# rounak-meyur/revs-admm

Measured on NVIDIA B200. Metric: home_hours_scheduled_per_sec, higher is better.
Workload: dtype f64

## Files before the change

revs-admm_b200/csrc/dual_update.cu:

```cuda
#include <cuda_bf16.h>

#include "kernels.cuh"

namespace revs {



__device__ __forceinline__ unsigned long long ld_acquire_sys(const unsigned long long* p) {
    unsigned long long v;
    asm volatile("ld.acquire.sys.global.u64 %0, [%1];" : "=l"(v) : "l"(p) : "memory");
    return v;
}
__device__ __forceinline__ void st_release_sys(unsigned long long* p, unsigned long long v) {
    asm volatile("st.release.sys.global.u64 [%0], %1;" ::"l"(p), "l"(v) : "memory");
}

template <int SLOTS, bool DSUM>
__global__ void __launch_bounds__(256, 4) dual_update_kernel(DualParams P) {
    extern __shared__ double tile[];
    __shared__ double s_part[2][8];
    const int lane = threadIdx.x & 31, warp = threadIdx.x >> 5;
    const int h0 = blockIdx.x * 32;
    const int ldt = P.T + 1;
    const int it = P.iter ? *P.iter : 0;
    const double* __restrict__ p_sch_new = (it & 1) ? P.p_sch_old : P.p_sch_new;
    const double* __restrict__ p_sch_old = (it & 1) ? P.p_sch_new : P.p_sch_old;
    double* __restrict__ diff_k = P.diff_k + (size_t)it * P.Hp;

    {
        const int h = h0 + lane;
        const bool in = h < P.Hp;
        const double* src = P.g_t + (in ? h : 0);
        int t = warp;
        for (; t + 24 < P.T; t += 32) {
            double v[4];
#pragma unroll
            for (int q = 0; q < 4; ++q) v[q] = in ? src[(size_t)(t + 8 * q) * P.Hp] : 0.0;
#pragma unroll
            for (int q = 0; q < 4; ++q) tile[lane * ldt + t + 8 * q] = v[q];
        }
        for (; t < P.T; t += 8) tile[lane * ldt + t] = in ? src[(size_t)t * P.Hp] : 0.0;
    }
    __syncthreads();

    const double hk = 0.5 * P.kappa;
    double blk_p = 0.0, blk_d = 0.0;
    const double* dsum = DSUM ? P.dsum : nullptr;
    if constexpr (SLOTS > 0) {
        for (int hl = warp; hl < 32; hl += 16) {
            double sn[2][SLOTS], gm[2][SLOTS], so[2][DSUM ? 1 : SLOTS];
            bool okh[2];
#pragma unroll
            for (int q = 0; q < 2; ++q) {
                const int h = h0 + hl + 8 * q;
                okh[q] = h < P.Hp;
                const size_t base = (size_t)(okh[q] ? h : 0) * P.T;
#pragma unroll
                for (int j = 0; j < SLOTS; ++j) {
// ... 59 lines not shown
            blk_p += a1;
            blk_d += a2;
        }
    }
    if (lane == 0) { s_part[0][warp] = blk_p; s_part[1][warp] = blk_d; }
    __syncthreads();

    __nv_bfloat16* gbf = reinterpret_cast<__nv_bfloat16*>(P.gbf_next);
    for (int t = warp; t < P.T; t += 8) {
        int h = h0 + lane;
        if (h < P.Hp) {
            const double zv = tile[lane * ldt + t];
            const size_t o = (size_t)t * P.Hp + h;
            P.z_t[o] = zv;
            if (P.g_next) {
                const double gv = fmax(zv, 0.0);
                P.g_next[o] = gv;
                if (gbf) gbf[o] = __float2bfloat16_rn((float)gv);
            }
        }
    }

    __shared__ int s_last;
    __shared__ double s_fin[2][8];
    if (threadIdx.x == 0) {
        double sp = 0.0, sd = 0.0;
        for (int w = 0; w < 8; ++w) { sp += s_part[0][w]; sd += s_part[1][w]; }
        P.partials[blockIdx.x] = sp;
        P.partials[gridDim.x + blockIdx.x] = sd;
        __threadfence();
        const unsigned done = atomicAdd(&P.res->ticket, 1u);
// ... 46 lines not shown
        if (P.peer.world > 1) {
            count = 0.0;
            for (int r = 0; r < P.peer.world; ++r) { tp += s_peer[0][r]; td += s_peer[1][r]; count += s_peer[2][r]; }
        } else {
            for (int w = 0; w < 8; ++w) { tp += s_fin[0][w]; td += s_fin[1][w]; }
        }
        const double r = sqrt(tp / count), sres = P.kappa * sqrt(td / count);
        const int conv = (P.tol > 0.0 && r < P.tol && sres < P.tol) ? 1 : 0;
        P.res->sum_primal = tp;
        P.res->sum_dual = td;
        P.res->count = count;
        P.res->primal = r;
        P.res->dual = sres;
        P.res->converged = conv;
        P.res->ticket = 0u;
        if (P.iter) {
            const int k = it + 1;
            *P.iter = k;
            if (P.use_cond) {
                const bool err = (P.err_a && *P.err_a) || (P.err_b && *P.err_b) || (P.peer.world > 1 && *P.peer.timeout);
                cudaGraphSetConditional((cudaGraphConditionalHandle)P.cond_loop, (k < P.iter_max && !conv && !err) ? 1u : 0u);
            }
        }
    }
}

cudaError_t launch_dual_update(const DualParams& P, cudaStream_t stream) {
    const size_t smem = (size_t)32 * (P.T + 1) * sizeof(double);
    const int slots = (P.T + 31) / 32;
    const dim3 grid((P.Hp + 31) / 32);
    auto go = [&](auto kernel) -> cudaError_t {
        if (smem > 48 * 1024) {
            cudaError_t e = cudaFuncSetAttribute(kernel, cudaFuncAttributeMaxDynamicSharedMemorySize, (int)smem);
            if (e != cudaSuccess) return e;
        }
        kernel<<<grid, 256, smem, stream>>>(P);
        return cudaGetLastError();
    };
    if (P.dsum) {
        switch (slots) {
            case 1: return go(dual_update_kernel<1, true>);
            case 2: return go(dual_update_kernel<2, true>);
            case 3: return go(dual_update_kernel<3, true>);
// ... 15 lines not shown
```

revs-admm_b200/csrc/home_solve.cu:

```cuda
#include <math_constants.h>

#include "kernels.cuh"

namespace revs {

constexpr int kMaxSlots = 8;
constexpr int kSelectRounds = 24;


template <int SLOTS>
__global__ void __launch_bounds__(256, SLOTS <= 3 ? 6 : 1) home_solve_kernel(HomeParams P) {
    const int lane = threadIdx.x & 31;
    const int h = blockIdx.x * (blockDim.x >> 5) + (threadIdx.x >> 5);
    if (h >= P.Hp) return;
    const size_t base = (size_t)h * P.T;
    const bool ev = P.has_ev[h] != 0;
    const double rate = P.rating[h];
    const int st = P.start[h], en = P.end[h];
    const int nmin = P.n_min[h], nmax = P.n_max[h];
    const bool odd = P.iter != nullptr && (*P.iter & 1);
    const double* __restrict__ p_sch_in = odd ? P.p_sch_new : P.p_sch;
    double* __restrict__ p_sch_out = odd ? const_cast<double*>(P.p_sch) : P.p_sch_new;

    double ld[SLOTS];
#pragma unroll
    for (int j = 0; j < SLOTS; ++j) {
        int t = lane + 32 * j;
        ld[j] = t < P.T ? P.load[base + t] : 0.0;
    }
    const bool first = P.iter ? (*P.iter == 0) : (P.first != 0);
    if (!ev) {
        double a2 = 0.0;
#pragma unroll
        for (int j = 0; j < SLOTS; ++j) {
            int t = lane + 32 * j;
            if (t < P.T) {
                p_sch_out[base + t] = ld[j];
                P.p_ev[base + t] = 0.0;
                const double ds = first ? ld[j] : 0.0;
                a2 = fma(ds, ds, a2);
            }
        }
        if (P.dsum) {
            a2 = warp_sum(a2);
            if (lane == 0) P.dsum[h] = a2;
// ... 99 lines not shown
#pragma unroll
                for (int j = 0; j < SLOTS; ++j) {
                    int t = lane + 32 * j;
                    rank[j] += (o < d[j]) || (o == d[j] && s < t);
                }
            }
        }
#pragma unroll
        for (int j = 0; j < SLOTS; ++j)
            on[j] = d[j] < CUDART_INF && (rank[j] < nmin || (rank[j] < nmax && d[j] < 0.0));
    }
    double a2 = 0.0;
#pragma unroll
    for (int j = 0; j < SLOTS; ++j) {
        int t = lane + 32 * j;
        if (t >= P.T) continue;
        double p = on[j] ? rate : 0.0;
        P.p_ev[base + t] = p;
        const double sn = __dadd_rn(ld[j], p);
        p_sch_out[base + t] = sn;
        const double ds = sn - prev[j];
        a2 = fma(ds, ds, a2);
    }
    if (P.dsum) {
        a2 = warp_sum(a2);
        if (lane == 0) P.dsum[h] = a2;
    }
}

cudaError_t launch_home_solve(const HomeParams& P, cudaStream_t stream) {
    const int warps = 8;
// ... 38 lines not shown
```

revs-admm_b200/csrc/kernels.cuh:

```cuda
#pragma once
#include <vector>

#include "common.cuh"

namespace revs {

struct HomeParams {
    const double* load;
    const double* p_est;
    const double* p_sch;
    const int* iter;
    const double* gamma;
    const double* cost;
    const uint8_t* has_ev;
    const double* rating;
    const int* start;
    const int* end;
    const int* n_min;
    const int* n_max;
    double* p_sch_new;
    double* p_ev;
    double* dsum;
    int first;
    int* infeasible;
    int Hp, T;
    double kappa;
    int individual;
    const double* ind_const;
};

cudaError_t launch_home_solve(const HomeParams& P, cudaStream_t stream);
cudaError_t launch_soc_profile(const double* p_ev, const uint8_t* has_ev, const double* capacity,
                               const double* initial, double* soc, int Hp, int T, cudaStream_t stream);

struct ResidualOut {
    double sum_primal;
    double sum_dual;
    double primal;
// ... 18 lines not shown
    const double* p_sch_old;
    const double* dsum;
    int* iter;
    int iter_max;
    int step;
    const int* err_a;
    const int* err_b;
    unsigned long long cond_loop;
    int use_cond;
    double* gamma;
    double* p_est;
    double* z_t;
    double* g_next;
    void* gbf_next;
    double* diff_k;
    ResidualOut* res;
    PeerReduce peer;
    double* partials;
    int Hp, T;
    double kappa, tol, count;
};

cudaError_t launch_dual_update(const DualParams& P, cudaStream_t stream);

struct QpParams {
    const FeederDev* feeders;
    const double* Rpool;
    const double* rn2;
    const double* rmax;
    int* cand;
// ... 51 lines not shown
cudaError_t launch_round_end(const RoundEndParams& P, cudaStream_t stream);

struct ClassGateParams {
    const int* order_count;
    unsigned long long cond[kQpClasses];
    int first_gated;
};
cudaError_t launch_class_gate(const ClassGateParams& P, cudaStream_t stream);
cudaError_t qp_warp_prepare();
cudaError_t screen_prepare();
cudaError_t screen_tc5_prepare();

cudaError_t launch_utility_qp(const QpParams& P, int grid, int cls, cudaStream_t stream);
int qp_warp_max_n();
cudaError_t launch_qp_init(const QpParams& P, int max_warp_n, cudaStream_t stream);
int qp_warp_ctas_per_sm();
int qp_warp_m_max_default();
cudaError_t launch_utility_qp_warp(const QpParams& P, int nj, int ctas_per_sm, cudaStream_t stream);
cudaError_t launch_utility_qp_fast(const QpParams& P, cudaStream_t stream);
cudaError_t launch_order_columns(const QpParams& P, int mode, int* order, int* order_count, cudaStream_t stream);

struct NewtonZone {
    int feeder;
    int nn, nlev, n;
    int wn;
    int col0;
    int64_t node_off;
    int64_t home_off;
    int64_t lvl_off;
    int64_t ws_off;
// ... 276 lines not shown
```

revs-admm_b200/csrc/revs_capi.cu:

```cuda
#include <chrono>
#include <cstdarg>
#include <cstdio>
#include <cstring>
#include <algorithm>
#include <cstdlib>
#include <cmath>
#include <mutex>
#include <string>
#include <vector>

#include "../../include/revs_admm.h"
#include "kernels.cuh"

using namespace revs;

namespace {

thread_local std::string g_err;

int fail(int code, const char* fmt, ...) {
    char buf[512];
    va_list ap;
    va_start(ap, fmt);
    vsnprintf(buf, sizeof buf, fmt, ap);
// ... 186 lines not shown
    double2* d_nt_ws2 = nullptr;
    int64_t nt_ws_stride = 0;
    int n_newton_cols = 0;
    size_t nt_sig = 0;
    double* d_gather = nullptr;
    int64_t gather_cap = 0;
    double* peer_gather[kGatherMaxPeers] = {};
    int gather_world = 1, gather_rank = 0;
    unsigned long long gather_seq = 0;
    GatherDev* d_gather_dev = nullptr;
    unsigned* d_gather_ticket = nullptr;
    int* d_gather_timeout = nullptr;
    bool use_warp_kernel = true;
    bool overlap_home = true;
    bool screen = true;
    int screen_impl = 0;
    void *d_maps_a = nullptr, *d_map_b = nullptr;
    int* d_bcol0 = nullptr;
    bool tc5_ready = false;
    int *d_pool_parent = nullptr, *d_pool_res = nullptr;
    double* d_pool_cumr = nullptr;
    int64_t* d_pool_off = nullptr;
    size_t pool_nodes = 0;
    NetTools net;
    size_t Rpool_elems = 0;
    bool rn2_valid = false;
    double *d_load = nullptr, *d_pest = nullptr, *d_psch[2] = {nullptr, nullptr}, *d_gamma = nullptr,
           *d_pev = nullptr, *d_soc = nullptr;
    uint8_t* d_has_ev = nullptr;
    double *d_rating = nullptr, *d_capacity = nullptr, *d_initial = nullptr, *d_indconst = nullptr;
// ... 548 lines not shown
        return fail(REVS_ERR_INFEASIBLE, "a home charging sub-problem is infeasible (SOC window vs plug-in window)");
    if (s->h_cnt->n_failed)
        return fail(REVS_ERR_NOCONV,
                    "utility QP: %d (feeder,hour) columns need more than %d simultaneously active "
                    "voltage rows", s->h_cnt->n_failed, kWMax);
    if (s->h_cnt->noconv)
        return fail(REVS_ERR_NOCONV, "utility QP: %d columns still running after %d working-set rounds (or a tree-Newton column "
                    "that did not reach the tolerance)", s->h_cnt->n_running, kQpRoundMax);
    return REVS_OK;
}

int utility_solve(revs_solver* s, bool in_loop = false) {
    int rc = prepare_sensitivity(s);
    if (rc) return rc;
    QpParams Q = qp_params(s);
    if ((rc = launch_init(s, Q, in_loop, true))) return rc;
    s->stats.kernel_launches++;
    if (newton_active(s)) {
        if ((rc = launch_newton_stage(s, true))) return rc;
        if (dense_cols(s) == 0) {
            CU(cudaMemcpyAsync(s->h_cnt, s->d_cnt, sizeof(Counters), cudaMemcpyDeviceToHost, s->sU));
            CU(cudaStreamSynchronize(s->sU));
            return check_device_flags(s);
        }
    }
    bool use[kQpClasses];
    for (int cl = 0; cl < kQpClasses; ++cl) use[cl] = cl <= 1 || qp_class_cap(cl - 1) < s->ws_bound;
    int top_cls = 0;
    int grid[kQpClasses];
    for (int cl = 0; cl < kQpClasses; ++cl) grid[cl] = s->ncols;
    for (int round = 0;; ++round) {
        if (round >= kQpRoundMax)
// ... 60 lines not shown
    P.rating = s->d_rating;
    P.start = s->d_start;
    P.end = s->d_end;
    P.n_min = individual ? s->d_zero_i : s->d_nmin;
    P.n_max = s->d_nmax;
    P.p_sch_new = s->d_psch[s->cur ^ 1];
    P.p_ev = s->d_pev;
    P.infeasible = &s->d_cnt->infeasible;
    P.Hp = (int)s->Hp;
    P.T = s->T;
    P.kappa = s->kappa;
    P.individual = individual;
    P.ind_const = s->d_indconst;
    P.dsum = nullptr;
    P.first = 0;
    return P;
}

void free_all(revs_solver* s) {
    cudaSetDevice(s->device);
    void* ptrs[] = {s->d_feeders, s->d_Rpool, s->d_rn2, s->d_rmax, s->d_cand, s->d_stage, s->d_hmap, s->d_Rbf, s->d_gbf, s->d_v32, s->d_sprob, s->d_stiles, s->d_maps_a, s->d_map_b, s->d_bcol0, s->d_pool_parent, s->d_pool_res, s->d_pool_cumr, s->d_pool_off, s->d_load, s->d_pest, s->d_psch[0], s->d_psch[1], s->d_gamma,
                    s->d_pev, s->d_soc, s->d_has_ev, s->d_rating, s->d_capacity, s->d_initial, s->d_indconst,
                    s->d_start, s->d_end, s->d_nmin, s->d_nmax, s->d_zero_i, s->d_cost, s->d_zt, s->d_lamt,
                    s->d_gt, s->d_vt, s->d_wcount, s->d_widx, s->d_status, s->d_innerok, s->d_cls, s->d_order, s->d_order4, s->d_order_count, s->d_cnt, s->d_diff,
                    s->d_cprob, s->d_ctiles, s->d_respart, s->d_dsum,
                    s->d_nt_zones, s->d_nt_lvl, s->d_nt_parent, s->d_nt_home, s->d_nt_hnode, s->d_nt_wsi, s->d_nt_child, s->d_nt_homes, s->d_nt_rho,
                    s->d_nt_ws, s->d_nt_ws4, s->d_nt_ws2};
    for (int r = 0; r < kMaxPeers; ++r)
        if (s->peer_box[r] && s->peer_box[r] != s->d_mailbox) cudaIpcCloseMemHandle(s->peer_box[r]);
    for (int r = 0; r < kGatherMaxPeers; ++r)
// ... 462 lines not shown
    D.cond_loop = 0;
    D.use_cond = 0;
    D.partials = s->d_respart;
    D.dsum = s->d_dsum;
    D.peer.world = s->comm_world;
    D.peer.rank = s->comm_rank;
    for (int r = 0; r < kMaxPeers; ++r) D.peer.box[r] = s->peer_box[r];
    D.peer.run_seq = s->d_run_seq;
    D.peer.timeout = s->d_comm_timeout;
    D.gamma = s->d_gamma;
    D.p_est = s->d_pest;
    D.z_t = s->d_zt;
    D.g_next = s->d_gt;
    D.gbf_next = s->screen ? s->d_gbf : nullptr;
    D.diff_k = s->d_diff;
    D.res = &s->d_cnt->res;
    D.Hp = (int)s->Hp;
    D.T = s->T;
    D.kappa = s->kappa;
    D.tol = s->tol;
    D.count = (double)s->H * s->T;
    return D;
}

int finish_sync(revs_solver* s, double sums[3]) {
    CU(cudaStreamSynchronize(s->sU));
    CU(cudaStreamSynchronize(s->sH));
    spans_collect(s);
    int rc = check_device_flags(s);
    if (rc == REVS_OK && s->comm_world > 1) {
// ... 17 lines not shown
        sums[2] = s->comm_world > 1 ? s->h_cnt->res.count : (double)s->H * s->T;
    }
    return REVS_OK;
}

int admm_step_impl(revs_solver* s, double sums[3], bool sync_now) {
    if (!s || !s->running) return fail(REVS_ERR_ARG, "revs_admm_begin has not been called");
    if (s->k >= s->iter_max) return fail(REVS_ERR_ARG, "iter_max iterations already done");
    CU(cudaSetDevice(s->device));

    cudaStream_t sHome = s->overlap_home ? s->sH : s->sU;
    CU(cudaStreamWaitEvent(sHome, s->evDualDone, 0));
    HomeParams hp = home_params(s, 0);
    hp.dsum = s->d_dsum;
    hp.first = s->k == 0 ? 1 : 0;
    TimedSpan* sp = span_begin(s, 1, sHome);
    CU(launch_home_solve(hp, sHome));
    span_end(sp, sHome);
    CU(cudaEventRecord(s->evHomeDone, sHome));
    s->stats.kernel_launches++;

    int rc = utility_solve(s, true);
    if (rc) { s->running = false; cudaDeviceSynchronize(); return rc; }

    CU(cudaStreamWaitEvent(s->sU, s->evHomeDone, 0));
    DualParams D = dual_params(s);
    D.p_sch_new = s->d_psch[s->cur ^ 1];
    D.p_sch_old = s->d_psch[s->cur];
    D.diff_k = s->d_diff + (size_t)s->k * s->Hp;
    sp = span_begin(s, 2, s->sU);
    CU(launch_dual_update(D, s->sU));
    span_end(sp, s->sU);
    s->stats.kernel_launches++;
    CU(cudaEventRecord(s->evDualDone, s->sU));
    CU(cudaMemcpyAsync(s->h_cnt, s->d_cnt, sizeof(Counters), cudaMemcpyDeviceToHost, s->sU));
    CU(cudaEventRecord(s->evT1, s->sU));
    s->cur ^= 1;
    s->k++;
    s->stats.admm_iterations = s->k;
    if (!sync_now) return REVS_OK;
    return finish_sync(s, sums);
}

int capture_loop(revs_solver* s) {
    const int flags = (s->screen ? 1 : 0) | (s->screen_impl << 1) | (s->overlap_home ? 4 : 0) | (s->use_warp_kernel ? 8 : 0) | (s->use_fast ? 16 : 0) | (s->comm_world << 8) | (s->comm_rank << 16) | (dense_cols(s) ? 64 : 0) | (newton_active(s) ? 128 : 0);
    if (s->loop_exec && s->gk_kappa == s->kappa && s->gk_vset == s->vset && s->gk_vhigh == s->vhigh && s->gk_tol == s->tol &&
        s->gk_iter_max == s->iter_max && s->gk_flags == flags)
        return REVS_OK;
    if (s->loop_exec) { cudaGraphExecDestroy(s->loop_exec); s->loop_exec = nullptr; }
    if (s->loop_graph) { cudaGraphDestroy(s->loop_graph); s->loop_graph = nullptr; }
    for (int cl = 1; cl < kQpClasses; ++cl) CU(launch_utility_qp(QpParams{}, 0, cl, s->sU));
    CU(qp_warp_prepare());
    CU(screen_prepare());
    CU(screen_tc5_prepare());
    CU(cudaGraphCreate(&s->loop_graph, 0));
    const bool rounds = dense_cols(s) > 0;
    cudaGraphConditionalHandle h_loop, h_round = 0;
    GateCapture gc{};
    CU(cudaGraphConditionalHandleCreate(&h_loop, s->loop_graph, 1, cudaGraphCondAssignDefault));
    if (rounds) {
        CU(cudaGraphConditionalHandleCreate(&h_round, s->loop_graph, 0, cudaGraphCondAssignDefault));
        for (int cl = 2; cl < kQpClasses; ++cl) CU(cudaGraphConditionalHandleCreate(&gc.h[cl], s->loop_graph, 0, cudaGraphCondAssignDefault));
    }
    cudaGraphNodeParams np_loop{};
    np_loop.type = cudaGraphNodeTypeConditional;
    np_loop.conditional.handle = h_loop;
    np_loop.conditional.type = cudaGraphCondTypeWhile;
    np_loop.conditional.size = 1;
    cudaGraphNode_t n_loop;
    CU(cudaGraphAddNode(&n_loop, s->loop_graph, nullptr, 0, &np_loop));
    cudaGraph_t body_loop = np_loop.conditional.phGraph_out[0];

    cudaGraph_t body_round = nullptr;
    CU(cudaStreamBeginCaptureToGraph(s->sU, body_loop, nullptr, nullptr, 0, cudaStreamCaptureModeRelaxed));
    int rc = REVS_OK;
    auto capture_body = [&]() -> int {
        cudaStream_t sHome = s->overlap_home ? s->sH : s->sU;
        if (s->overlap_home) {
            CU(cudaEventRecord(s->evV, s->sU));
            CU(cudaStreamWaitEvent(s->sH, s->evV, 0));
        }
        HomeParams hp = home_params(s, 0);
        hp.p_sch = s->d_psch[0];
        hp.p_sch_new = s->d_psch[1];
        hp.iter = &s->d_cnt->iter;
        hp.dsum = s->d_dsum;
        CU(launch_home_solve(hp, sHome));
        if (s->overlap_home) CU(cudaEventRecord(s->evHomeDone, s->sH));
        QpParams Q = qp_params(s);
        if (rounds) {
            Q.cond_round = (unsigned long long)h_round;
            Q.use_cond = 1;
        }
        int r = launch_init(s, Q, true, false);
        if (r) return r;
        if (newton_active(s)) {
            const revs_stats keep = s->stats;
            r = launch_newton_stage(s, false);
            s->stats = keep;
            if (r) return r;
        }
        if (rounds) {
            cudaStreamCaptureStatus st;
            cudaGraph_t g_cap = nullptr;
            const cudaGraphNode_t* deps = nullptr;
            size_t n_deps = 0;
            CU(cudaStreamGetCaptureInfo(s->sU, &st, nullptr, &g_cap, &deps, &n_deps));
            cudaGraphNodeParams np_round{};
            np_round.type = cudaGraphNodeTypeConditional;
            np_round.conditional.handle = h_round;
            np_round.conditional.type = cudaGraphCondTypeWhile;
            np_round.conditional.size = 1;
            cudaGraphNode_t n_round;
            CU(cudaGraphAddNode(&n_round, g_cap, deps, n_deps, &np_round));
            body_round = np_round.conditional.phGraph_out[0];
            CU(cudaStreamUpdateCaptureDependencies(s->sU, &n_round, 1, cudaStreamSetCaptureDependencies));
        }
        if (s->overlap_home) CU(cudaStreamWaitEvent(s->sU, s->evHomeDone, 0));
        DualParams D = dual_params(s);
        D.iter = &s->d_cnt->iter;
        D.cond_loop = (unsigned long long)h_loop;
        D.use_cond = 1;
        CU(launch_dual_update(D, s->sU));
        return REVS_OK;
    };
    rc = capture_body();
    cudaGraph_t got = nullptr;
    cudaError_t ce = cudaStreamEndCapture(s->sU, &got);
    if (rc) return rc;
    if (ce != cudaSuccess) return fail(REVS_ERR_CUDA, "capture of the ADMM loop body failed: %s", cudaGetErrorString(ce));
    if (rounds) {
        CU(cudaStreamBeginCaptureToGraph(s->sU, body_round, nullptr, nullptr, 0, cudaStreamCaptureModeRelaxed));
        auto capture_round = [&]() -> int {
            QpParams Q = qp_params(s);
            const revs_stats keep = s->stats;
            int r = enqueue_round(s, Q, -1, nullptr, nullptr, false, &gc);
            s->stats = keep;
// ... 33 lines not shown

int revs_admm_step(revs_solver* s, double sums[3]) { return admm_step_impl(s, sums, true); }

int revs_solve_admm(revs_solver* s, double kappa, int iter_max, double vset, double vlow, double vhigh,
                    double tol, int* iters_done) {
    const double th0 = now_ms();
    int rc = revs_admm_begin(s, kappa, iter_max, vset, vlow, vhigh);
    if (rc) return rc;
    s->host_sync_ms = 0.0;
    for (double& v : s->cat_ms) v = 0.0;
    const double th1 = now_ms();
    s->tol = tol;
    if (s->use_graph) {
        if ((rc = prepare_sensitivity(s))) return rc;
        if ((rc = capture_loop(s))) { s->tol = 0.0; return rc; }
        CU(cudaGraphLaunch(s->loop_exec, s->sU));
        CU(cudaMemcpyAsync(s->h_cnt, s->d_cnt, sizeof(Counters), cudaMemcpyDeviceToHost, s->sU));
        CU(cudaEventRecord(s->evT1, s->sU));
        CU(cudaEventRecord(s->evDualDone, s->sU));
        rc = finish_sync(s, nullptr);
        s->tol = 0.0;
        s->k = s->h_cnt->iter;
        s->cur = s->k & 1;
        s->stats.admm_iterations = s->k;
        s->stats.qp_outer_iterations = (int64_t)s->h_cnt->rounds_total;
        s->stats.gemm_launches = (int64_t)s->h_cnt->rounds_total;
        s->stats.gemm_full_launches = s->k;
        s->stats.qp_warp_rounds = (s->use_warp_kernel && s->zg.warp_n > 0) ? (int64_t)s->h_cnt->rounds_total : 0;
        s->stats.kernel_launches += (int64_t)s->k * (newton_active(s) ? 4 : 3) + (int64_t)s->h_cnt->rounds_total * round_launches(s);
        if (rc) return rc;
    } else {
        for (int k = 0; k < iter_max; ++k) {
            rc = admm_step_impl(s, nullptr, tol > 0.0 || k == iter_max - 1);
            if (rc) { s->tol = 0.0; return rc; }
            if (tol > 0.0 && s->h_cnt->res.converged) break;
        }
        s->tol = 0.0;
    }
    if (s->debug_host)
        fprintf(stderr, "[revs host] dev %d: begin %.3f ms, loop %.3f ms (waiting in round syncs %.3f ms), device span %.3f ms, %s | "
                "span sums: screen %.2f+%.2f home %.2f dual %.2f cls1 %.2f cls2-3 %.2f init %.2f warp-mid/big %.2f warp-small %.2f\n",
                s->device, th1 - th0, now_ms() - th1, s->host_sync_ms, s->stats.total_ms, s->use_graph ? "captured loop" : "host-driven loop",
                s->cat_ms[5], s->cat_ms[0], s->cat_ms[1], s->cat_ms[2], s->cat_ms[3], s->cat_ms[4], s->cat_ms[6], s->cat_ms[7], s->cat_ms[8]);
    if (iters_done) *iters_done = s->k;
// ... 1031 lines not shown
    if (!s || !name) return fail(REVS_ERR_ARG, "bad arguments");
    const bool mid_run = s->running && s->k > 0 && s->k < s->iter_max;
    if (!strcmp(name, "screen")) {
        if (value != 0.0 && s->zg.max_n > kScreenMaxN)
            return fail(REVS_ERR_ARG, "screening is limited to zones of at most %d residences", kScreenMaxN);
        if (mid_run) return fail(REVS_ERR_ARG, "'screen' cannot change between revs_admm_step calls of one run");
        s->screen = value != 0.0;
        return REVS_OK;
    }
    if (!strcmp(name, "newton_min_n")) {
        for (int f = 0; f < s->nf; ++f)
            if (s->sens_set[f]) return fail(REVS_ERR_ARG, "set option 'newton_min_n' before the feeders are given");
        s->newton_min_n = value < 0.0 ? 0 : (value > 2e9 ? 2000000000 : (int)value);
        return REVS_OK;
    }
    if (!strcmp(name, "graph")) { s->use_graph = value != 0.0; return REVS_OK; }
    if (!strcmp(name, "warp_kernel")) { s->use_warp_kernel = value != 0.0; return REVS_OK; }
    if (!strcmp(name, "overlap_home")) { s->overlap_home = value != 0.0; return REVS_OK; }
    if (!strcmp(name, "priority")) {
        CU(cudaSetDevice(s->device));
        CU(cudaStreamSynchronize(s->sU));
        int pr = s->prio_hi + (int)value;
        if (pr > s->prio_lo - 1) pr = s->prio_lo - 1;
        if (pr < s->prio_hi) pr = s->prio_hi;
        CU(cudaStreamDestroy(s->sU));
        CU(cudaStreamCreateWithPriority(&s->sU, cudaStreamNonBlocking, pr));
        for (int cl = 0; cl < kQpClasses; ++cl) {
            CU(cudaStreamSynchronize(s->sQ[cl]));
            CU(cudaStreamDestroy(s->sQ[cl]));
            CU(cudaStreamCreateWithPriority(&s->sQ[cl], cudaStreamNonBlocking, pr));
// ... 19 lines not shown
```

revs-admm_b200/csrc/utility_qp.cu:

```cuda
#include <algorithm>

#include <cuda_bf16.h>

#include "kernels.cuh"

namespace revs {

constexpr int kJT = 64;
constexpr int kTld = kJT + 1;
constexpr double kArcMin = 9.5367431640625e-07;
constexpr int kChgMax = 128;
constexpr int kMaskWords = 512;
constexpr int kPdasMax = 40;
constexpr double kHessShift = 1e-12;

template <int WMAX, int THREADS>
struct QpSmem {
    double Hb[WMAX * (WMAX + 1)];
    double tileR[WMAX * kTld];
    double hdiag[WMAX];
    double lam[WMAX], trial[WMAX], grad[WMAX], dir[WMAX], b[WMAX], y[WMAX];
    double red[3 * (THREADS / 32)];
    double bcast[2];
    int idx[WMAX], fl[WMAX], inA[WMAX];
// ... 565 lines not shown
            if (lane == 0) { sm.red[warp] = best; sm.ired[warp] = besti; }
            __syncthreads();
            best = sm.red[0]; besti = sm.ired[0];
#pragma unroll
            for (int w = 1; w < THREADS / 32; ++w) {
                if (sm.red[w] > best || (sm.red[w] == best && sm.ired[w] < besti)) { best = sm.red[w]; besti = sm.ired[w]; }
            }
            if (best < 0.0) break;
            if (round == room) { n_viol_left = 1; break; }
            if (tid == 0) { sm.idx[m + added] = besti; sm.lam[m + added] = 0.0; }
            ++added;
            prev_v = best; prev_i = besti;
        }
        __syncthreads();
        if (added == 0 && n_viol_left == 0 && inner_prev == 1) {
            if (tid == 0) P.status[c] = 1;
            finished = true;
            break;
        }
        if (n_viol_left && m + added == WMAX) {
            if (!BIG) {
                if (tid == 0) {
                    P.cls[c] = CLS + 1;
                    P.inner_ok[c] = (pass > 0 || inner_prev == 3) ? 3 : 2;
                    atomicAdd(P.n_running, 1);
                    atomicAdd(P.n_cls + CLS + 1, 1);
                }
                handed = true;
                break;
            }
            if (added == 0) {
// ... 178 lines not shown
                if (found || tau > 1e40 || mf == 0) break;
                tau *= 1e3;
            }
            if (alpha == 1.0) tau = fmax(1.0, tau / 10.0);
        }
        PHASE(3);
        __syncthreads();
        for (int a = tid; a < m; a += THREADS) sm.lam[a] = sm.trial[a];
        __syncthreads();
        phi = eval_phi<THREADS>(R, ld, n, z, sm.idx, sm.lam, m, u, g, sm, nullptr, nullptr, nullptr, gbf);
        flops += 2.0 * m * n;
        PHASE(4);
    }

    __syncthreads();
    for (int a = tid; a < m; a += THREADS) {
        lam_g[sm.idx[a]] = sm.lam[a];
        widx[a] = sm.idx[a];
    }
    const bool done = clean && ok && its == 0;
    its_all += (unsigned long long)its;
    if (tid == 0) {
        P.wcount[c] = m;
        P.inner_ok[c] = ok;
        P.status[c] = done ? 1 : 0;
    }
    if (done) { finished = true; break; }
    if (!self_verify || !ok || inner_max <= 0) break;
    __syncthreads();
    exact_voltages<THREADS>(R, ld, n, g, v);
    flops += 2.0 * n * n;
    inner_prev = 1;
    }

    if (tid == 0) {
        if (!finished && !handed) { atomicAdd(P.n_running, 1); atomicAdd(P.n_cls + CLS, 1); }
        atomicAdd(P.newton_its, its_all);
        atomicAdd(P.cols, 1ull);
// ... 142 lines not shown
```

revs-admm_b200/csrc/utility_qp_warp.cu:

```cuda
#include <cstdlib>

#include <cuda_bf16.h>

#include "kernels.cuh"

namespace revs {

namespace {

#ifndef REVS_WARPS_PER_CTA
#define REVS_WARPS_PER_CTA 4
#endif
constexpr int kWarpsPerCta = REVS_WARPS_PER_CTA;
constexpr int kCtasPerSm = 16 / kWarpsPerCta;
constexpr int kHW = kWW + 1;
constexpr int kCacheDoubles = 1024;
constexpr double kArcMinW = 9.5367431640625e-07;
constexpr int kPdasMaxW = 40;
constexpr double kHessShiftW = 1e-12;
constexpr int kAddMaxW = 8;
constexpr int kPassMaxW = 10;
constexpr int kRecheckMaxW = 256;
constexpr int kHysteresisW = 8;

// ... 566 lines not shown
        if (lane < m_old) lam_g[wi] = 0.0;
        __syncwarp();
        if (lane < m) { lam_g[idx] = lam; widx[lane] = idx; }
        if (changed) {
            __nv_bfloat16* gbf = P.gbf_t ? reinterpret_cast<__nv_bfloat16*>(P.gbf_t) + col : nullptr;
#pragma unroll
            for (int k = 0; k < NJ; ++k) {
                const int j = lane + 32 * k;
                if (j < n) {
                    g[j] = gj[k];
                    if (gbf) gbf[j] = __float2bfloat16_rn((float)gj[k]);
                }
            }
        }
    }
    if (lane == 0) {
        P.wcount[c] = m;
        P.inner_ok[c] = 1;
        if (exit_kind == 0) P.status[c] = 1;
    }
    if (exit_kind == 1) ++st.deferred;
    trace_out(exit_kind);
    st.its += (unsigned long long)its_total;
    st.flops += flops;
    st.max_ws = max(st.max_ws, m);
#undef WPHASE
}

}

__global__ void __launch_bounds__(256) qp_init_kernel(QpParams P, int max_warp_n) {
    const int lane = threadIdx.x & 31;
// ... 11 lines not shown
        return;
    }
    const double* R = P.Rpool + fd.roff;
    const size_t col = (size_t)t * P.Hp + fd.off;
    const double* z = P.z_t + col;
    double* lam_g = P.lam_t + col;
    double* g = P.g_t + col;
    __nv_bfloat16* gbf = P.gbf_t ? reinterpret_cast<__nv_bfloat16*>(P.gbf_t) + col : nullptr;
    int* widx = P.widx + (size_t)c * kWMax;

    int m = 0;
    if (P.init == 2) {
        const int wc = P.wcount[c];
        if (wc == 0) {
            if (lane == 0) {
                P.cls[c] = n <= max_warp_n ? 0 : 1;
                P.status[c] = 0;
                P.inner_ok[c] = 0;
                if (P.cand) P.cand[c] = 0;
            }
            return;
        }
        for (int a0 = 0; a0 < wc; a0 += 32) {
            const int a = a0 + lane;
            const int i = a < wc ? widx[a] : 0;
            const bool on = a < wc && lam_g[i] > 0.0;
            const unsigned bal = __ballot_sync(0xffffffffu, on);
            __syncwarp();
            if (on) widx[m + __popc(bal & ((1u << lane) - 1))] = i;
            m += __popc(bal);
        }
    } else {
        for (int j0 = 0; j0 < n; j0 += 32) {
            const int j = j0 + lane;
            const bool on = j < n && lam_g[j] > 0.0;
            const unsigned bal = __ballot_sync(0xffffffffu, on);
            if (on) {
                const int pos = m + __popc(bal & ((1u << lane) - 1));
                if (pos < kWMax) widx[pos] = j;
                else lam_g[j] = 0.0;
            }
            m += __popc(bal);
        }
        m = min(m, kWMax);
    }
    __syncwarp();
    int cl = (n <= max_warp_n && m <= (n <= 128 ? P.warp_m_max : P.warp_m_max_big)) ? 0 : 1;
    while (cl < kQpClasses - 1 && m > qp_class_cap(cl)) ++cl;

    for (int j0 = 0; j0 < n; j0 += 32) {
        const int j = j0 + lane;
        if (j >= n) break;
        double pi = 0.0;
        for (int a = 0; a < m; ++a) {
            const int i = widx[a];
            pi = fma(R[(size_t)i * ld + j], lam_g[i], pi);
        }
        const double gj = fmax(z[j] - pi, 0.0);
        g[j] = gj;
        if (gbf) gbf[j] = __float2bfloat16_rn((float)gj);
    }
    if (lane == 0) {
        P.wcount[c] = m;
// ... 212 lines not shown
        }
        recheck_rows<NJ>(candk, R, ld, n, gj, vub);
        bool viol = false;
#pragma unroll
        for (int k = 0; k < NJ; ++k) {
            const int j = lane + 32 * k;
            viol |= j < n && j != i0 && vub[k] - u > tol;
        }
        if (__any_sync(full, viol)) { pass_on(); continue; }

        const bool changed = (i0 >= 0) && (l != lam_old || nviol == 1);
        const int m_new = i0 >= 0 ? 1 : 0;
        if (lane == 0) {
            if (m_old == 1) lam_g[w0] = 0.0;
            if (i0 >= 0) { lam_g[i0] = l; widx[0] = i0; }
            P.wcount[c] = m_new;
            P.inner_ok[c] = 1;
            P.status[c] = 1;
        }
        if (changed) {
            double* g = P.g_t + col;
            __nv_bfloat16* gbf = P.gbf_t ? reinterpret_cast<__nv_bfloat16*>(P.gbf_t) + col : nullptr;
#pragma unroll
            for (int k = 0; k < NJ; ++k) {
                const int j = lane + 32 * k;
                if (j < n) {
                    g[j] = gj[k];
                    if (gbf) gbf[j] = __float2bfloat16_rn((float)gj[k]);
                }
            }
            its_sum += (unsigned long long)its;
// ... 82 lines not shown
```

Measured before the change: 267.8 million.

## Fold QP warm-start init into dual update and window home solve to charging hours

Moves the per-iteration QP initialisation (class/status reset and projected g = max(z - R^T lam, 0) from the previous active set) into the dual-update kernel, removing one kernel launch per ADMM iteration inside the graph. The QP kernels now store a compacted active set with only positive multipliers, so the folded init can skip the recompaction step. The home solve also skips non-EV homes and non-window hours after the first iteration. The cost is extra shared memory, extra global reads in the dual-update kernel, and a more complex conditional-graph setup.

After: 272.9 million (median of 6 runs). 1.9% higher.

```diff
diff --git a/profiles/exp_fold_init.py b/profiles/exp_fold_init.py
--- /dev/null
+++ b/profiles/exp_fold_init.py
@@ -0,0 +1,150 @@
+import argparse
+import filecmp
+import hashlib
+import json
+import os
+import shutil
+import statistics
+import subprocess
+import sys
+import time
+
+ROOT = os.path.dirname(os.path.dirname(os.path.abspath(__file__)))
+WORKLOAD = "synthetic-refshape-125k-homes-per-gpu-x96"
+
+
+def _problem():
+    sys.path.insert(0, ROOT)
+    import bench
+    return bench, bench.make_rank_problem(WORKLOAD, 0)
+
+
+def solve_worker(opts, steps):
+    import numpy as np
+    import torch
+    bench, (trees, hm, cost, sizes, T) = _problem()
+    import revs_admm_b200 as R
+    with R.PipelinedSolver(sizes, T, pipelines=4) as s:
+        for k, v in opts.items():
+            s.set_option(k, v)
+        s.set_feeder_trees(trees)
+        s.set_homes(**hm)
+        s.set_tariff(cost)
+        for _ in range(3):
+            s.solve_admm(**bench.ADMM)
+        torch.cuda.synchronize()
+        ms = []
+        for _ in range(steps):
+            t0 = time.perf_counter()
+            s.solve_admm(**bench.ADMM)
+            torch.cuda.synchronize()
+            ms.append((time.perf_counter() - t0) * 1e3)
+        out = s.results()
+        out["P_est"], out["Gamma"] = s.estimate()
+    digest = {k: hashlib.sha256(np.ascontiguousarray(v).tobytes()).hexdigest()[:16] for k, v in sorted(out.items())}
+    print(json.dumps({"ms_per_step": statistics.median(ms), "ms": ms, "sha": digest}))
+
+
+def spans_worker():
+    import numpy as np
+    bench, (trees, hm, cost, sizes, T) = _problem()
+    import revs_admm_b200 as R
+    rows = []
+    with R.Solver(sizes, T) as s:
+        s.set_option("graph", 0)
+        s.set_option("overlap_home", 0)
+        s.set_feeder_trees(trees)
+        s.set_homes(**hm)
+        s.set_tariff(cost)
+        for i in range(5):
+            s.solve_admm(**bench.ADMM)
+            st = s.stats()
+            if i >= 2:
+                rows.append({k: float(st[k]) for k in ("qp_init_ms", "dual_ms", "home_ms", "total_ms")})
+    print(json.dumps({k: float(np.median([r[k] for r in rows])) for k in rows[0]}))
+
+
+def gpu_info():
+    q = "name,power.limit,clocks.sm,clocks.max.sm"
+    out = subprocess.run(["nvidia-smi", f"--query-gpu={q}", "--format=csv,noheader"], capture_output=True, text=True).stdout
+    return dict(zip(q.split(","), [x.strip() for x in out.strip().splitlines()[0].split(",")])) if out.strip() else None
+
+
+def last_json(text):
+    for line in reversed(text.strip().splitlines()):
+        if line.startswith("{"):
+            return json.loads(line)
+    raise RuntimeError("no JSON line in:\n" + text[-3000:])
+
+
+def run(cmd, lib):
+    env = dict(os.environ, REVS_LIB=os.path.abspath(lib))
+    r = subprocess.run(cmd, cwd=ROOT, env=env, capture_output=True, text=True)
+    if r.returncode != 0:
+        raise RuntimeError(" ".join(cmd) + "\n" + r.stdout[-3000:] + r.stderr[-3000:])
+    return last_json(r.stdout)
+
+
+def main():
+    ap = argparse.ArgumentParser()
+    ap.add_argument("--lib-a", required=True, help="parent build")
+    ap.add_argument("--lib-b", required=True, help="this build")
+    ap.add_argument("--out", required=True)
+    ap.add_argument("--rounds", type=int, default=2, help="alternations of the solve-worker configurations")
+    ap.add_argument("--steps", type=int, default=10)
+    ap.add_argument("--bench", type=int, default=0, help="pairs of bench.py runs (parent, this build)")
+    ap.add_argument("--worker", default=None, help=argparse.SUPPRESS)
+    args = ap.parse_args()
+    if args.worker == "spans":
+        return spans_worker()
+    if args.worker is not None:
+        return solve_worker(json.loads(args.worker), args.steps)
+    os.makedirs(args.out, exist_ok=True)
+    me = os.path.abspath(__file__)
+    res = {"gpu_before": gpu_info(), "solve": {}, "bench": {"a": [], "b": []}, "spans": {}}
+    configs = [("parent", args.lib_a, {}), ("off", args.lib_b, {"fold_init": 0, "home_window": 0}),
+               ("fold_init", args.lib_b, {"fold_init": 1, "home_window": 0}),
+               ("home_window", args.lib_b, {"fold_init": 0, "home_window": 1}), ("both", args.lib_b, {})]
+    for r in range(args.rounds):
+        for name, lib, opts in configs:
+            o = run([sys.executable, me, "--lib-a", "-", "--lib-b", "-", "--out", "-", "--steps", str(args.steps),
+                     "--worker", json.dumps(opts)], lib)
+            res["solve"].setdefault(name, []).append(o)
+            print(name, r, round(o["ms_per_step"], 3), flush=True)
+    ref = res["solve"]["parent"][0]["sha"]
+    res["solve_mismatches"] = {name: sorted({k for o in runs for k, v in o["sha"].items() if ref[k] != v})
+                               for name, runs in res["solve"].items()}
+    res["solve_ms_median"] = {name: statistics.median(o["ms_per_step"] for o in runs) for name, runs in res["solve"].items()}
+    for p in range(args.bench):
+        for tag, lib in (("a", args.lib_a), ("b", args.lib_b)):
+            d = os.path.join(args.out, f"dump_{tag}{p}")
+            line = run([sys.executable, "bench.py", "--gpus", "1", "--steps", str(args.steps), "--warmup", "3",
+                        "--no-cpu-baseline", "--no-exact", "--no-convergence", "--dump-outputs", d], lib)
+            res["bench"][tag].append({"device_ms_per_step": line.get("device_ms_per_step"),
+                                      "e2e_ms_per_step": line.get("e2e", {}).get("ms_per_step"),
+                                      "ms_per_step": line.get("ms_per_step")})
+            print(tag, p, res["bench"][tag][-1], flush=True)
+    if args.bench:
+        refd = os.path.join(args.out, "dump_a0")
+        names = sorted(os.listdir(refd))
+        res["dump_mismatches"] = [f"{t}{p}/{n}" for t in "ab" for p in range(args.bench) for n in names
+                                  if not filecmp.cmp(os.path.join(refd, n), os.path.join(args.out, f"dump_{t}{p}", n), shallow=False)]
+        for t in "ab":
+            for p in range(args.bench):
+                shutil.rmtree(os.path.join(args.out, f"dump_{t}{p}"), ignore_errors=True)
+        gains = [1.0 - b["device_ms_per_step"] / a["device_ms_per_step"] for a, b in zip(res["bench"]["a"], res["bench"]["b"])]
+        res["bench_device_gain_per_pair"] = gains
+        res["bench_e2e_gain_per_pair"] = [1.0 - b["e2e_ms_per_step"] / a["e2e_ms_per_step"]
+                                          for a, b in zip(res["bench"]["a"], res["bench"]["b"])]
+    for tag, lib in (("parent", args.lib_a), ("this", args.lib_b)):
+        res["spans"][tag] = run([sys.executable, me, "--lib-a", "-", "--lib-b", "-", "--out", "-", "--worker", "spans"], lib)
+        print(tag, "spans", res["spans"][tag], flush=True)
+    res["gpu_after"] = gpu_info()
+    with open(os.path.join(args.out, "exp_fold_init.json"), "w") as f:
+        json.dump(res, f, indent=1)
+    print(json.dumps({k: res.get(k) for k in ("gpu_before", "solve_ms_median", "solve_mismatches", "bench_device_gain_per_pair",
+                                              "bench_e2e_gain_per_pair", "dump_mismatches")}))
+
+
+if __name__ == "__main__":
+    main()
diff --git a/revs-admm_b200/csrc/dual_update.cu b/revs-admm_b200/csrc/dual_update.cu
--- a/revs-admm_b200/csrc/dual_update.cu
+++ b/revs-admm_b200/csrc/dual_update.cu
@@ -4,7 +4,7 @@
 
 namespace revs {
 
-
+constexpr int kStartPairs = 4;
 
 __device__ __forceinline__ unsigned long long ld_acquire_sys(const unsigned long long* p) {
     unsigned long long v;
@@ -27,6 +27,43 @@
     const double* __restrict__ p_sch_old = (it & 1) ? P.p_sch_new : P.p_sch_old;
     double* __restrict__ diff_k = P.diff_k + (size_t)it * P.Hp;
 
+    const bool start = P.feeders != nullptr;
+    double* s_lam = tile + 32 * ldt;
+    int* s_idx = reinterpret_cast<int*>(s_lam + 2 * P.T * kStartPairs);
+    int* s_wc = s_idx + 2 * P.T * kStartPairs;
+    __shared__ FeederDev s_fd[2];
+    __shared__ int s_zone[2];
+    if (start) {
+        if (warp == 0) {
+            int lo = 0, hi = P.nf;
+            while (hi - lo > 1) {
+                const int step = (hi - lo + 31) / 32;
+                const int k = lo + lane * step;
+                const unsigned bal = __ballot_sync(0xffffffffu, k < hi && P.feeders[k].off <= h0);
+                lo += (31 - __clz(bal)) * step;
+                hi = min(hi, lo + step);
+            }
+            if (lane < 2) {
+                const int f = lo + lane;
+                const bool on = f < P.nf && (lane == 0 || P.feeders[f].off < h0 + 32);
+                s_zone[lane] = on ? f : -1;
+                if (on) s_fd[lane] = P.feeders[f];
+            }
+        }
+        const int ncols = P.nf * P.T;
+        for (int c = blockIdx.x * blockDim.x + threadIdx.x; c < ncols; c += gridDim.x * blockDim.x) {
+            const FeederDev fd = P.feeders[c / P.T];
+            if (fd.roff < 0) {
+                P.cls[c] = 0; P.status[c] = 1; P.inner_ok[c] = 1;
+            } else {
+                const int wc = P.wcount[c];
+                P.cls[c] = qp_start_class(fd.n, wc, wc, P.max_warp_n, P.warp_m_max, P.warp_m_max_big);
+                P.status[c] = 0; P.inner_ok[c] = 0;
+            }
+            if (P.cand) P.cand[c] = 0;
+        }
+    }
+
     {
         const int h = h0 + lane;
         const bool in = h < P.Hp;
@@ -42,6 +79,24 @@
         for (; t < P.T; t += 8) tile[lane * ldt + t] = in ? src[(size_t)t * P.Hp] : 0.0;
     }
     __syncthreads();
+    if (start) {
+        for (int i = threadIdx.x; i < 2 * P.T; i += blockDim.x) {
+            const int q = i >= P.T, t = i - q * P.T, f = s_zone[q];
+            int wc = 0;
+            if (f >= 0 && s_fd[q].roff >= 0) {
+                const int c = f * P.T + t;
+                wc = P.wcount[c];
+                int idx[kStartPairs];
+#pragma unroll
+                for (int a = 0; a < kStartPairs; ++a) idx[a] = a < wc ? P.widx[(size_t)c * kWMax + a] : 0;
+                const double* lam = P.lam_t + (size_t)t * P.Hp + s_fd[q].off;
+#pragma unroll
+                for (int a = 0; a < kStartPairs; ++a)
+                    if (a < wc) { s_idx[i * kStartPairs + a] = idx[a]; s_lam[i * kStartPairs + a] = lam[idx[a]]; }
+            }
+            s_wc[i] = wc;
+        }
+    }
 
     const double hk = 0.5 * P.kappa;
     double blk_p = 0.0, blk_d = 0.0;
@@ -131,7 +186,32 @@
             const size_t o = (size_t)t * P.Hp + h;
             P.z_t[o] = zv;
             if (P.g_next) {
-                const double gv = fmax(zv, 0.0);
+                double pi = 0.0;
+                if (start) {
+                    const int q = s_zone[1] >= 0 && h >= s_fd[1].off;
+                    const int i = q * P.T + t, wc = s_wc[i];
+                    const FeederDev& fd = s_fd[q];
+                    const int j = h - (int)fd.off;
+                    if (wc > 0 && j < fd.n) {
+                        const double* Rj = P.Rpool + fd.roff + j;
+                        const double* lam = P.lam_t + (size_t)t * P.Hp + fd.off;
+                        const int* widx = P.widx + (size_t)(s_zone[q] * P.T + t) * kWMax;
+                        for (int a0 = 0; a0 < wc; a0 += kStartPairs) {
+                            double r[kStartPairs], l[kStartPairs];
+#pragma unroll
+                            for (int u = 0; u < kStartPairs; ++u) {
+                                const int a = a0 + u;
+                                const int ri = a0 == 0 ? s_idx[i * kStartPairs + u] : (a < wc ? widx[a] : 0);
+                                l[u] = a0 == 0 ? s_lam[i * kStartPairs + u] : (a < wc ? lam[ri] : 0.0);
+                                r[u] = a < wc ? Rj[(size_t)ri * fd.np] : 0.0;
+                            }
+#pragma unroll
+                            for (int u = 0; u < kStartPairs; ++u)
+                                if (a0 + u < wc) pi = fma(r[u], l[u], pi);
+                        }
+                    }
+                }
+                const double gv = fmax(zv - pi, 0.0);
                 P.g_next[o] = gv;
                 if (gbf) gbf[o] = __float2bfloat16_rn((float)gv);
             }
@@ -208,6 +288,10 @@
         P.res->dual = sres;
         P.res->converged = conv;
         P.res->ticket = 0u;
+        if (P.round_ctr) {
+            *P.round_ctr = 0;
+            if (P.use_cond) cudaGraphSetConditional((cudaGraphConditionalHandle)P.cond_round, 1u);
+        }
         if (P.iter) {
             const int k = it + 1;
             *P.iter = k;
@@ -220,7 +304,8 @@
 }
 
 cudaError_t launch_dual_update(const DualParams& P, cudaStream_t stream) {
-    const size_t smem = (size_t)32 * (P.T + 1) * sizeof(double);
+    const size_t smem = (size_t)32 * (P.T + 1) * sizeof(double) +
+                        (P.feeders ? (size_t)2 * P.T * (kStartPairs * (sizeof(double) + sizeof(int)) + sizeof(int)) : 0);
     const int slots = (P.T + 31) / 32;
     const dim3 grid((P.Hp + 31) / 32);
     auto go = [&](auto kernel) -> cudaError_t {
diff --git a/revs-admm_b200/csrc/home_solve.cu b/revs-admm_b200/csrc/home_solve.cu
--- a/revs-admm_b200/csrc/home_solve.cu
+++ b/revs-admm_b200/csrc/home_solve.cu
@@ -21,14 +21,26 @@
     const bool odd = P.iter != nullptr && (*P.iter & 1);
     const double* __restrict__ p_sch_in = odd ? P.p_sch_new : P.p_sch;
     double* __restrict__ p_sch_out = odd ? const_cast<double*>(P.p_sch) : P.p_sch_new;
+    const bool first = P.iter ? (*P.iter == 0) : (P.first != 0);
+    const bool win = P.window && !first;
+    if (win && !ev) {
+        if (P.dsum && lane == 0) P.dsum[h] = 0.0;
+        return;
+    }
 
     double ld[SLOTS];
 #pragma unroll
     for (int j = 0; j < SLOTS; ++j) {
         int t = lane + 32 * j;
-        ld[j] = t < P.T ? P.load[base + t] : 0.0;
-    }
-    const bool first = P.iter ? (*P.iter == 0) : (P.first != 0);
+        ld[j] = t < P.T && (!win || (t >= st && t < en)) ? P.load[base + t] : 0.0;
+    }
+    if (P.window && first) {
+#pragma unroll
+        for (int j = 0; j < SLOTS; ++j) {
+            int t = lane + 32 * j;
+            if (t < P.T && !(ev && t >= st && t < en)) const_cast<double*>(p_sch_in)[base + t] = ld[j];
+        }
+    }
     if (!ev) {
         double a2 = 0.0;
 #pragma unroll
@@ -158,7 +170,7 @@
 #pragma unroll
     for (int j = 0; j < SLOTS; ++j) {
         int t = lane + 32 * j;
-        if (t >= P.T) continue;
+        if (t >= P.T || (win && (t < st || t >= en))) continue;
         double p = on[j] ? rate : 0.0;
         P.p_ev[base + t] = p;
         const double sn = __dadd_rn(ld[j], p);
diff --git a/revs-admm_b200/csrc/kernels.cuh b/revs-admm_b200/csrc/kernels.cuh
--- a/revs-admm_b200/csrc/kernels.cuh
+++ b/revs-admm_b200/csrc/kernels.cuh
@@ -22,6 +22,7 @@
     double* p_ev;
     double* dsum;
     int first;
+    int window;
     int* infeasible;
     int Hp, T;
     double kappa;
@@ -70,6 +71,19 @@
     double* g_next;
     void* gbf_next;
     double* diff_k;
+    const FeederDev* feeders;
+    int nf;
+    const double* Rpool;
+    const double* lam_t;
+    const int* wcount;
+    const int* widx;
+    int* cls;
+    int* status;
+    int* inner_ok;
+    int* cand;
+    int max_warp_n, warp_m_max, warp_m_max_big;
+    int* round_ctr;
+    unsigned long long cond_round;
     ResidualOut* res;
     PeerReduce peer;
     double* partials;
@@ -151,6 +165,12 @@
 cudaError_t launch_utility_qp(const QpParams& P, int grid, int cls, cudaStream_t stream);
 int qp_warp_max_n();
 cudaError_t launch_qp_init(const QpParams& P, int max_warp_n, cudaStream_t stream);
+__device__ __forceinline__ int qp_start_class(int n, int wc, int m, int max_warp_n, int warp_m_max, int warp_m_max_big) {
+    if (wc == 0) return n <= max_warp_n ? 0 : 1;
+    int cl = (n <= max_warp_n && m <= (n <= 128 ? warp_m_max : warp_m_max_big)) ? 0 : 1;
+    while (cl < kQpClasses - 1 && m > qp_class_cap(cl)) ++cl;
+    return cl;
+}
 int qp_warp_ctas_per_sm();
 int qp_warp_m_max_default();
 cudaError_t launch_utility_qp_warp(const QpParams& P, int nj, int ctas_per_sm, cudaStream_t stream);
diff --git a/revs-admm_b200/csrc/revs_capi.cu b/revs-admm_b200/csrc/revs_capi.cu
--- a/revs-admm_b200/csrc/revs_capi.cu
+++ b/revs-admm_b200/csrc/revs_capi.cu
@@ -224,6 +224,8 @@
     bool use_warp_kernel = true;
     bool overlap_home = true;
     bool screen = true;
+    bool fold_init = true;
+    bool home_window = true;
     int screen_impl = 0;
     void *d_maps_a = nullptr, *d_map_b = nullptr;
     int* d_bcol0 = nullptr;
@@ -802,8 +804,10 @@
     int rc = prepare_sensitivity(s);
     if (rc) return rc;
     QpParams Q = qp_params(s);
-    if ((rc = launch_init(s, Q, in_loop, true))) return rc;
-    s->stats.kernel_launches++;
+    if (!in_loop || !s->fold_init || s->k == 0) {
+        if ((rc = launch_init(s, Q, in_loop, true))) return rc;
+        s->stats.kernel_launches++;
+    }
     if (newton_active(s)) {
         if ((rc = launch_newton_stage(s, true))) return rc;
         if (dense_cols(s) == 0) {
@@ -894,6 +898,7 @@
     P.ind_const = s->d_indconst;
     P.dsum = nullptr;
     P.first = 0;
+    P.window = 0;
     return P;
 }
 
@@ -1386,6 +1391,21 @@
     D.g_next = s->d_gt;
     D.gbf_next = s->screen ? s->d_gbf : nullptr;
     D.diff_k = s->d_diff;
+    if (s->fold_init) {
+        D.feeders = s->d_feeders;
+        D.nf = s->nf;
+        D.Rpool = s->d_Rpool;
+        D.lam_t = s->d_lamt;
+        D.wcount = s->d_wcount;
+        D.widx = s->d_widx;
+        D.cls = s->d_cls;
+        D.status = s->d_status;
+        D.inner_ok = s->d_innerok;
+        D.cand = s->screen ? s->d_cand : nullptr;
+        D.max_warp_n = s->use_warp_kernel ? qp_warp_max_n() : 0;
+        D.warp_m_max = s->warp_m_max;
+        D.warp_m_max_big = s->warp_m_max_big;
+    }
     D.res = &s->d_cnt->res;
     D.Hp = (int)s->Hp;
     D.T = s->T;
@@ -1433,6 +1453,7 @@
     HomeParams hp = home_params(s, 0);
     hp.dsum = s->d_dsum;
     hp.first = s->k == 0 ? 1 : 0;
+    hp.window = s->home_window ? 1 : 0;
     TimedSpan* sp = span_begin(s, 1, sHome);
     CU(launch_home_solve(hp, sHome));
     span_end(sp, sHome);
@@ -1462,7 +1483,7 @@
 }
 
 int capture_loop(revs_solver* s) {
-    const int flags = (s->screen ? 1 : 0) | (s->screen_impl << 1) | (s->overlap_home ? 4 : 0) | (s->use_warp_kernel ? 8 : 0) | (s->use_fast ? 16 : 0) | (s->comm_world << 8) | (s->comm_rank << 16) | (dense_cols(s) ? 64 : 0) | (newton_active(s) ? 128 : 0);
+    const int flags = (s->screen ? 1 : 0) | (s->screen_impl << 1) | (s->overlap_home ? 4 : 0) | (s->use_warp_kernel ? 8 : 0) | (s->use_fast ? 16 : 0) | (s->comm_world << 8) | (s->comm_rank << 16) | (dense_cols(s) ? 64 : 0) | (newton_active(s) ? 128 : 0) | (s->fold_init ? 32 : 0) | (s->home_window ? 1 << 24 : 0);
     if (s->loop_exec && s->gk_kappa == s->kappa && s->gk_vset == s->vset && s->gk_vhigh == s->vhigh && s->gk_tol == s->tol &&
         s->gk_iter_max == s->iter_max && s->gk_flags == flags)
         return REVS_OK;
@@ -1478,7 +1499,7 @@
     GateCapture gc{};
     CU(cudaGraphConditionalHandleCreate(&h_loop, s->loop_graph, 1, cudaGraphCondAssignDefault));
     if (rounds) {
-        CU(cudaGraphConditionalHandleCreate(&h_round, s->loop_graph, 0, cudaGraphCondAssignDefault));
+        CU(cudaGraphConditionalHandleCreate(&h_round, s->loop_graph, s->fold_init ? 1 : 0, cudaGraphCondAssignDefault));
         for (int cl = 2; cl < kQpClasses; ++cl) CU(cudaGraphConditionalHandleCreate(&gc.h[cl], s->loop_graph, 0, cudaGraphCondAssignDefault));
     }
     cudaGraphNodeParams np_loop{};
@@ -1504,6 +1525,7 @@
         hp.p_sch_new = s->d_psch[1];
         hp.iter = &s->d_cnt->iter;
         hp.dsum = s->d_dsum;
+        hp.window = s->home_window ? 1 : 0;
         CU(launch_home_solve(hp, sHome));
         if (s->overlap_home) CU(cudaEventRecord(s->evHomeDone, s->sH));
         QpParams Q = qp_params(s);
@@ -1511,7 +1533,7 @@
             Q.cond_round = (unsigned long long)h_round;
             Q.use_cond = 1;
         }
-        int r = launch_init(s, Q, true, false);
+        int r = s->fold_init ? REVS_OK : launch_init(s, Q, true, false);
         if (r) return r;
         if (newton_active(s)) {
             const revs_stats keep = s->stats;
@@ -1540,6 +1562,10 @@
         D.iter = &s->d_cnt->iter;
         D.cond_loop = (unsigned long long)h_loop;
         D.use_cond = 1;
+        if (s->fold_init && rounds) {
+            D.round_ctr = &s->d_cnt->round;
+            D.cond_round = (unsigned long long)h_round;
+        }
         CU(launch_dual_update(D, s->sU));
         return REVS_OK;
     };
@@ -1603,6 +1629,7 @@
     if (s->use_graph) {
         if ((rc = prepare_sensitivity(s))) return rc;
         if ((rc = capture_loop(s))) { s->tol = 0.0; return rc; }
+        if (s->fold_init && (rc = launch_init(s, qp_params(s), true, false))) { s->tol = 0.0; return rc; }
         CU(cudaGraphLaunch(s->loop_exec, s->sU));
         CU(cudaMemcpyAsync(s->h_cnt, s->d_cnt, sizeof(Counters), cudaMemcpyDeviceToHost, s->sU));
         CU(cudaEventRecord(s->evT1, s->sU));
@@ -1616,7 +1643,8 @@
         s->stats.gemm_launches = (int64_t)s->h_cnt->rounds_total;
         s->stats.gemm_full_launches = s->k;
         s->stats.qp_warp_rounds = (s->use_warp_kernel && s->zg.warp_n > 0) ? (int64_t)s->h_cnt->rounds_total : 0;
-        s->stats.kernel_launches += (int64_t)s->k * (newton_active(s) ? 4 : 3) + (int64_t)s->h_cnt->rounds_total * round_launches(s);
+        s->stats.kernel_launches += (int64_t)s->k * (2 + (newton_active(s) ? 1 : 0) + (s->fold_init ? 0 : 1)) + (s->fold_init ? 1 : 0) +
+                                    (int64_t)s->h_cnt->rounds_total * round_launches(s);
         if (rc) return rc;
     } else {
         for (int k = 0; k < iter_max; ++k) {
@@ -2678,6 +2706,11 @@
         s->newton_min_n = value < 0.0 ? 0 : (value > 2e9 ? 2000000000 : (int)value);
         return REVS_OK;
     }
+    if (!strcmp(name, "fold_init") || !strcmp(name, "home_window")) {
+        if (mid_run) return fail(REVS_ERR_ARG, "'%s' cannot change between revs_admm_step calls of one run", name);
+        (name[0] == 'f' ? s->fold_init : s->home_window) = value != 0.0;
+        return REVS_OK;
+    }
     if (!strcmp(name, "graph")) { s->use_graph = value != 0.0; return REVS_OK; }
     if (!strcmp(name, "warp_kernel")) { s->use_warp_kernel = value != 0.0; return REVS_OK; }
     if (!strcmp(name, "overlap_home")) { s->overlap_home = value != 0.0; return REVS_OK; }
diff --git a/revs-admm_b200/csrc/utility_qp.cu b/revs-admm_b200/csrc/utility_qp.cu
--- a/revs-admm_b200/csrc/utility_qp.cu
+++ b/revs-admm_b200/csrc/utility_qp.cu
@@ -603,7 +603,11 @@
         }
         __syncthreads();
         if (added == 0 && n_viol_left == 0 && inner_prev == 1) {
-            if (tid == 0) P.status[c] = 1;
+            if (tid == 0) {
+                for (int a = 0; a < m; ++a) widx[a] = sm.idx[a];
+                P.wcount[c] = m;
+                P.status[c] = 1;
+            }
             finished = true;
             break;
         }
@@ -812,14 +816,20 @@
     }
 
     __syncthreads();
+    const bool done = clean && ok && its == 0;
     for (int a = tid; a < m; a += THREADS) {
         lam_g[sm.idx[a]] = sm.lam[a];
-        widx[a] = sm.idx[a];
-    }
-    const bool done = clean && ok && its == 0;
+        if (!done) widx[a] = sm.idx[a];
+    }
     its_all += (unsigned long long)its;
     if (tid == 0) {
-        P.wcount[c] = m;
+        int ms = m;
+        if (done) {
+            ms = 0;
+            for (int a = 0; a < m; ++a)
+                if (sm.lam[a] > 0.0) widx[ms++] = sm.idx[a];
+        }
+        P.wcount[c] = ms;
         P.inner_ok[c] = ok;
         P.status[c] = done ? 1 : 0;
     }
diff --git a/revs-admm_b200/csrc/utility_qp_warp.cu b/revs-admm_b200/csrc/utility_qp_warp.cu
--- a/revs-admm_b200/csrc/utility_qp_warp.cu
+++ b/revs-admm_b200/csrc/utility_qp_warp.cu
@@ -604,8 +604,15 @@
             }
         }
     }
+    int m_stored = m;
+    if (exit_kind == 0) {
+        const unsigned keep = __ballot_sync(0xffffffffu, lane < m && lam > 0.0);
+        __syncwarp();
+        if ((keep >> lane) & 1u) widx[__popc(keep & ((1u << lane) - 1))] = idx;
+        m_stored = __popc(keep);
+    }
     if (lane == 0) {
-        P.wcount[c] = m;
+        P.wcount[c] = m_stored;
         P.inner_ok[c] = 1;
         if (exit_kind == 0) P.status[c] = 1;
     }
@@ -647,7 +654,7 @@
         const int wc = P.wcount[c];
         if (wc == 0) {
             if (lane == 0) {
-                P.cls[c] = n <= max_warp_n ? 0 : 1;
+                P.cls[c] = qp_start_class(n, 0, 0, max_warp_n, P.warp_m_max, P.warp_m_max_big);
                 P.status[c] = 0;
                 P.inner_ok[c] = 0;
                 if (P.cand) P.cand[c] = 0;
@@ -678,8 +685,7 @@
         m = min(m, kWMax);
     }
     __syncwarp();
-    int cl = (n <= max_warp_n && m <= (n <= 128 ? P.warp_m_max : P.warp_m_max_big)) ? 0 : 1;
-    while (cl < kQpClasses - 1 && m > qp_class_cap(cl)) ++cl;
+    const int cl = qp_start_class(n, 1, m, max_warp_n, P.warp_m_max, P.warp_m_max_big);
 
     for (int j0 = 0; j0 < n; j0 += 32) {
         const int j = j0 + lane;
@@ -922,7 +928,7 @@
         if (lane == 0) {
             if (m_old == 1) lam_g[w0] = 0.0;
             if (i0 >= 0) { lam_g[i0] = l; widx[0] = i0; }
-            P.wcount[c] = m_new;
+            P.wcount[c] = (i0 >= 0 && l > 0.0) ? 1 : 0;
             P.inner_ok[c] = 1;
             P.status[c] = 1;
         }
```
